# mila-iqia/babyai

Hardware: AMD Instinct MI355X
Metric: env-steps/sec (higher is better)
Workload: dtype u8; 1 GPU; BabyAI-BossLevel-v0 56x56x3 pixel (RGBImgPartialObsWrapper) obs, 1048576 envs in total = 1048576 per GPU x 1, random actions, auto-reset; envs_per_gpu=1048576, total_envs=1048576, parallelism=env-shards x1, no collective

## Files before the change

babyai_amd/csrc/bbai_engine.hip:

```cpp
#include <hip/hip_runtime.h>
#include <stdio.h>
#include <string.h>
#include <stdlib.h>
#include <algorithm>
#include <vector>

#if defined(BBAI_BOT_PROF)
__device__ unsigned long long g_bot_prof[32];
#endif
#include "../../include/bbai.h"
#include "bbai_types.hpp"
#include "bbai_kernels.hpp"
#include "bbai_gen.hpp"
#include "bbai_genl.hpp"
#include "bbai_step.hpp"
#include "bbai_view.hpp"
#include "bbai_grid.hpp"
#include "bbai_bot.hpp"
#include "bbai_seed.hpp"

using namespace bbai;

static_assert(sizeof(bbai_level_cfg) == sizeof(LevelCfg), "C ABI cfg mirrors bbai::LevelCfg");

// ... 79 lines not shown
    hipEvent_t ev_refill[NWIN];
    int gate_strict;
    volatile uint32_t* host_flags;
    uint32_t* host_flags_dev;
    hipStream_t probed[8];
    bool probed_ok[8];
    int n_probed;
    int gate_probe;
    int gate_forced;
    hipStream_t last_stream;
    bool have_stream;
    hipEvent_t ev_switch;
    bool call_events;
    int render_tpb;
    int render_group;
    int pregen_cap;
    int pregen_per_group;
    int pregen_min;
    int pregen_group;
    unsigned long long* tap_mask; uint32_t* tap_rank0; int32_t* tap_perm; int64_t* tap_ids; int64_t tap_count;
    uint32_t* mtt;
    uint8_t* mtpar;
    uint8_t* lane_tmpl;
    int lane_words;
    int pregen_lane;
    int lane_blocks;
    int step_prio;
    bool prof_on;
    struct ProfSlot { hipEvent_t a, b; bool used; } prof[3][PROF_RING];
    int prof_pos[3];
    double prof_ms[3];
    int64_t prof_n[3];
    int64_t prof_step_ticks;
    int rollout_multi;
    int64_t tick;
    uint8_t* vplane;
    uint16_t* fcache;
    uint8_t* cplane;
    uint8_t* lsm;
    unsigned int* render_tickets;
    int render_queue;
    int render_queue_bpc;
    int render_queue_blocks;
    int render_pace;
    uint8_t* rt_pixels;
    uint8_t* rt_shadow;
    bool rt_valid;
    int64_t rt_filled;
    int render_delta;
    int render_delta_sched;
    int render_delta_tpb;
    int render_delta_bpc;
    uint64_t* rt_dmask;
    int render_delta_from_step;
    int n_cus;
    int done_action_enum;
    int consume_fused;
    int inplace;
    uint8_t* atlas;
    uint8_t* lut;
    int n_tiles;
    uint8_t* grid_atlas[3];
    uint8_t* grid_lut[3];
    int grid_tiles[3];
    int grid_bpc;
    bool seeded, live;
    uint8_t* bot_state;
    int bot_stack;
    uint16_t* bot_work;
    uint32_t* bot_rows;
    int bot_group;
    int bot_eager;
    int64_t bot_threads;
    uint64_t* bot_stats;
};

typedef uint32_t u32x4 __attribute__((ext_vector_type(4)));
__device__ __forceinline__ void count_resets(unsigned long long* __restrict__ totals, unsigned int k, unsigned int blk) {
    atomicAdd(&totals[(blk & (SHARDS - 1)) * SHARD_U64], (unsigned long long)k);
}
constexpr int STEP_BLOCK = 64;
#ifndef BBAI_STEP_WAVES
#define BBAI_STEP_WAVES 1
#endif
#ifndef BBAI_PREFETCH_ID
#define BBAI_PREFETCH_ID 0
#endif

#ifndef BBAI_VIEW_LDS
#define BBAI_VIEW_LDS 0
#endif
__device__ __forceinline__ void window_fetch(const uint32_t* __restrict__ q, int rstride, uint32_t* wd) {
#pragma unroll
    for (int r = 0; r < VIEW; ++r) { wd[3 * r] = q[r * rstride]; wd[3 * r + 1] = q[r * rstride + 1]; wd[3 * r + 2] = q[r * rstride + 2]; }
}
__device__ __forceinline__ void view_cells(const uint32_t* wd, int off, int dir, uint32_t ce, int nfe,
                                           uint8_t* __restrict__ scr , uint32_t* cp, uint32_t* vis, int& fe2) {
    uint32_t* win = (uint32_t*)scr;
#pragma unroll
    for (int r = 0; r < VIEW; ++r) {
        win[2 * r] = __builtin_amdgcn_alignbyte(wd[3 * r + 1], wd[3 * r], off);
        win[2 * r + 1] = __builtin_amdgcn_alignbyte(wd[3 * r + 2], wd[3 * r + 1], off);
    }
    const int k0 = dir == 0 ? 6 : dir == 1 ? 54 : dir == 2 ? 48 : 0;
    const int kvi = dir == 0 ? 8 : dir == 1 ? -1 : dir == 2 ? -8 : 1;
    const int kvj = dir == 0 ? -1 : dir == 1 ? -8 : dir == 2 ? 1 : 8;
// ... 1174 lines not shown
    if (threadIdx.x == 0) {
        const unsigned int t0 = atomicAdd(counter, 1u);
        s_ticket[0] = t0;
        s_origin = __builtin_amdgcn_s_memrealtime() * 160ull - ((unsigned long long)t0 * NC + cidx) * (unsigned long long)pace_x16;
    }
    __syncthreads();
    for (;;) {
        const int64_t sg = (int64_t)s_ticket[tp] * NC + cidx;
        if (sg >= n_super) break;
        if (pace_x16) {
            const unsigned long long due = s_origin + (unsigned long long)sg * (unsigned long long)pace_x16;
            while (__builtin_amdgcn_s_memrealtime() * 160ull < due) __builtin_amdgcn_s_sleep(1);
        }
#pragma unroll
        for (int kk = 0; kk < K; ++kk) {
            const int64_t grp = sg * K + kk;
            if (grp >= all_groups) break;
            const int64_t env0 = grp * RENDER_GROUP;
            const int ne = (int)(n - env0 < RENDER_GROUP ? n - env0 : RENDER_GROUP);
            for (int c = threadIdx.x; c < ne * VIEW * VIEW; c += RENDER_BLOCK) {
                const int e = c / (VIEW * VIEW), cell = c - e * (VIEW * VIEW);
                const uint8_t* o = image + (env0 + e) * OBS_BYTES + cell * 3;
                const int key = o[0] | (o[1] << 3) | (o[2] << 6);
                s_tile[buf][c] = s_lut[(cell == 3 * VIEW + 6 ? 256 : 0) + key];
                if (shadow) shadow[env0 * (VIEW * VIEW) + c] = s_tile[buf][c];
            }
            if (kk == 0 && threadIdx.x == 0) s_ticket[tp ^ 1] = atomicAdd(counter, 1u);
            __syncthreads();
            u32x4* out = (u32x4*)(pixels + env0 * PIX_BYTES);
            for (int q = threadIdx.x; q < ne * VEC_PER_ENV; q += RENDER_BLOCK) {
                const int e = q / VEC_PER_ENV, k = q - e * VEC_PER_ENV;
                const uint8_t* t49 = s_tile[buf] + e * (VIEW * VIEW);
                const uint64_t lo = render_chunk(s_atlas, t49, 2 * k);
                const uint64_t hi = render_chunk(s_atlas, t49, 2 * k + 1);
                u32x4 v = {(uint32_t)lo, (uint32_t)(lo >> 32), (uint32_t)hi, (uint32_t)(hi >> 32)};
                __builtin_nontemporal_store(v, out + q);
            }
            buf ^= 1;
        }
        tp ^= 1;
    }
    if (threadIdx.x == 0) {
        unsigned int* departed = counters + 64 * NC;
        if (atomicAdd(departed, 1u) == gridDim.x - 1) {
            for (int c = 0; c <= NC; ++c) atomicExch(counters + 64 * c, 0u);
        }
    }
}

constexpr int LINE_BYTES = 128;
constexpr int DELTA_UNIT = 8;
constexpr int UNIT_LINES = DELTA_UNIT * PIX_BYTES / LINE_BYTES;
static_assert(DELTA_UNIT * PIX_BYTES % LINE_BYTES == 0 && PIX_BYTES % 64 == 0, "8-env units are whole 128-byte lines");

__device__ __forceinline__ uint64_t line_cells(int s, int t) {
    uint64_t m = 0;
    for (int b = s; b < t; b += 8) {
        const int ch = b >> 3, py = ch / CHUNKS_PER_ROW, cx = ch - py * CHUNKS_PER_ROW;
        m |= 1ull << ((cx / 3) * VIEW + (py >> 3));
    }
    return m;
}

template <int G, int T, int SCHED>
__global__ __launch_bounds__(T) void k_render_delta(int64_t n, const uint8_t* __restrict__ image, uint8_t* __restrict__ pixels,
                                                    uint8_t* __restrict__ shadow ,
                                                    const uint8_t* __restrict__ atlas, const uint8_t* __restrict__ lut, int n_tiles) {
    static_assert(G % DELTA_UNIT == 0 && T % 64 == 0 && G % (T / 64) == 0, "whole units per group, whole envs per wave");
    constexpr int W = T / 64, EPW = G / W, GL = G / DELTA_UNIT * UNIT_LINES;
    __shared__ __attribute__((aligned(16))) uint8_t s_atlas[MAX_TILES * TILE_BYTES];
    __shared__ uint64_t s_lma[UNIT_LINES], s_lmb[UNIT_LINES];
    __shared__ uint8_t s_lea[UNIT_LINES];
    __shared__ uint64_t s_dmask[2][G];
    __shared__ uint8_t s_lut[512];
    __shared__ uint8_t s_tile[2][G * CELLS + 8];
    __shared__ uint16_t s_list[2][GL];
    __shared__ unsigned int s_nd[2];
    for (int k = threadIdx.x; k < n_tiles * TILE_BYTES / 8; k += T) ((uint64_t*)s_atlas)[k] = ((const uint64_t*)atlas)[k];
    for (int k = threadIdx.x; k < 512; k += T) s_lut[k] = lut[k];
    for (int l = threadIdx.x; l < UNIT_LINES; l += T) {
        const int b0 = l * LINE_BYTES, b1 = b0 + LINE_BYTES;
        const int ea = b0 / PIX_BYTES, eb = (b1 - 1) / PIX_BYTES;
        s_lea[l] = (uint8_t)ea;
        s_lma[l] = line_cells(b0 - ea * PIX_BYTES, (eb != ea ? (ea + 1) * PIX_BYTES : b1) - ea * PIX_BYTES);
        s_lmb[l] = eb != ea ? line_cells(0, b1 - eb * PIX_BYTES) : 0;
    }
    const int lane = threadIdx.x & 63, wave = threadIdx.x >> 6;
    const int64_t ngroups = (n + G - 1) / G;
    int64_t g, gend, gstep;
    if (SCHED == 0) { g = blockIdx.x; gend = ngroups; gstep = gridDim.x; }
    else { const int64_t per = (ngroups + gridDim.x - 1) / gridDim.x; g = blockIdx.x * per; gend = g + per < ngroups ? g + per : ngroups; gstep = 1; }
    uint32_t o0[EPW], o1[EPW], o2[EPW], old[EPW];
    auto load = [&](int64_t grp) {
#pragma unroll
        for (int j = 0; j < EPW; ++j) {
            const int64_t env = grp * G + wave + j * W;
            o0[j] = o1[j] = o2[j] = old[j] = 0;
            if (grp < gend && lane < CELLS && env < n) {
                const uint8_t* o = image + env * OBS_BYTES + lane * 3;
                o0[j] = o[0]; o1[j] = o[1]; o2[j] = o[2];
                old[j] = shadow[env * CELLS + lane];
            }
        }
    };
    load(g);
    __syncthreads();
    int buf = 0;
    for (; g < gend; g += gstep, buf ^= 1) {
        const int64_t env0 = g * G;
        const int ne = (int)(n - env0 < G ? n - env0 : G);
#pragma unroll
        for (int j = 0; j < EPW; ++j) {
            const int e = wave + j * W;
            const bool live = lane < CELLS && e < ne;
            const int key = o0[j] | (o1[j] << 3) | (o2[j] << 6);
            const uint32_t id = live ? s_lut[(lane == AGENT_CELL ? 256 : 0) + key] : 0;
            const bool d = live && id != old[j];
            const uint64_t m = __ballot(d);
            if (live) s_tile[buf][e * CELLS + lane] = (uint8_t)id;
            if (d) shadow[(env0 + e) * CELLS + lane] = (uint8_t)id;
            if (lane == 0) s_dmask[buf][e] = m;
        }
        if (threadIdx.x == 0) s_nd[buf] = 0;
        __syncthreads();
        const int nl = (int)(((int64_t)ne * PIX_BYTES + LINE_BYTES - 1) / LINE_BYTES);
        for (int L0 = threadIdx.x - lane; L0 < nl; L0 += T) {
            const int L = L0 + lane;
            bool d = false;
            if (L < nl) {
                const int u = L / UNIT_LINES, l = L - u * UNIT_LINES, ea = u * DELTA_UNIT + s_lea[l];
                d = ((s_dmask[buf][ea] & s_lma[l]) | (s_lmb[l] ? s_dmask[buf][ea + 1] & s_lmb[l] : 0)) != 0;
            }
            const uint64_t m = __ballot(d);
            if (!m) continue;
            unsigned int base = 0;
            if (lane == 0) base = atomicAdd(&s_nd[buf], (unsigned int)__builtin_popcountll(m));
            base = __shfl(base, 0);
            if (d) s_list[buf][base + __builtin_popcountll(m & ((1ull << lane) - 1))] = (uint16_t)L;
        }
        __syncthreads();
        const int64_t gn = g + gstep;
        load(gn);
        const int nq = ne * VEC_PER_ENV, nd8 = (int)s_nd[buf] * 8;
        u32x4* out = (u32x4*)(pixels + env0 * PIX_BYTES);
        for (int i = threadIdx.x; i < nd8; i += T) {
            const int q = (int)s_list[buf][i >> 3] * 8 + (i & 7);
            if (q >= nq) continue;
            const int e = q / VEC_PER_ENV, k = q - e * VEC_PER_ENV;
            const uint8_t* t49 = s_tile[buf] + e * CELLS;
            const uint64_t lo = render_chunk(s_atlas, t49, 2 * k);
            const uint64_t hi = render_chunk(s_atlas, t49, 2 * k + 1);
            u32x4 v = {(uint32_t)lo, (uint32_t)(lo >> 32), (uint32_t)hi, (uint32_t)(hi >> 32)};
            __builtin_nontemporal_store(v, out + q);
        }
    }
}

constexpr int DSTORE_PIECES = 32 * CELLS / 8;
template <int G, int T>
__global__ __launch_bounds__(T) void k_render_dstore(int64_t n, uint8_t* __restrict__ pixels, const uint8_t* __restrict__ shadow ,
                                                     const uint64_t* __restrict__ dmask , const uint8_t* __restrict__ atlas, int n_tiles) {
    static_assert(G == 32 && T >= DSTORE_PIECES && T >= G && T % 64 == 0, "one 8-byte shadow piece per thread and group");
    constexpr int GL = G / DELTA_UNIT * UNIT_LINES;
    __shared__ __attribute__((aligned(16))) uint8_t s_atlas[MAX_TILES * TILE_BYTES];
    __shared__ uint64_t s_lma[UNIT_LINES], s_lmb[UNIT_LINES];
    __shared__ uint8_t s_lea[UNIT_LINES];
    __shared__ uint64_t s_dmask[2][G];
    __shared__ __attribute__((aligned(8))) uint8_t s_tile[2][G * CELLS + 8];
    __shared__ uint16_t s_list[2][GL];
    __shared__ unsigned int s_nd[2];
    for (int k = threadIdx.x; k < n_tiles * TILE_BYTES / 8; k += T) ((uint64_t*)s_atlas)[k] = ((const uint64_t*)atlas)[k];
    for (int l = threadIdx.x; l < UNIT_LINES; l += T) {
        const int b0 = l * LINE_BYTES, b1 = b0 + LINE_BYTES;
        const int ea = b0 / PIX_BYTES, eb = (b1 - 1) / PIX_BYTES;
        s_lea[l] = (uint8_t)ea;
        s_lma[l] = line_cells(b0 - ea * PIX_BYTES, (eb != ea ? (ea + 1) * PIX_BYTES : b1) - ea * PIX_BYTES);
        s_lmb[l] = eb != ea ? line_cells(0, b1 - eb * PIX_BYTES) : 0;
    }
    const int tid = threadIdx.x, lane = tid & 63;
    const int64_t ngroups = (n + G - 1) / G;
    const int64_t gstep = gridDim.x;
    int64_t g = blockIdx.x;
    auto load_mask = [&](int64_t grp) -> uint64_t {
        const int64_t env = grp * G + tid;
        return (tid < G && grp < ngroups && env < n) ? dmask[env] : 0ull;
    };
    const uint64_t shared_a = line_cells(PIX_BYTES - LINE_BYTES / 2, PIX_BYTES), shared_b = line_cells(0, LINE_BYTES / 2);
    static_assert(PIX_BYTES % LINE_BYTES == LINE_BYTES / 2, "two envs of a pair share one line");
    auto drawn = [&](int b, int e, int c0, int c1) -> bool {
        if (s_dmask[b][e]) return true;
        const uint64_t pm = (c1 == 63 ? ~0ull : (2ull << c1) - 1) & ~((1ull << c0) - 1);
        const bool shared_stored = ((s_dmask[b][e & ~1] & shared_a) | (s_dmask[b][e | 1] & shared_b)) != 0;
        return shared_stored && (pm & ((e & 1) ? shared_b : shared_a)) != 0;
    };
    auto load_ids = [&](int64_t grp, int b) -> uint2 {
        uint2 r = make_uint2(0u, 0u);
        if (tid >= DSTORE_PIECES || grp >= ngroups) return r;
        const int b0 = 8 * tid, b1 = b0 + 7, ea = b0 / CELLS, eb = b1 / CELLS;
        const bool need = eb == ea ? drawn(b, ea, b0 - ea * CELLS, b1 - ea * CELLS) : (drawn(b, ea, b0 - ea * CELLS, CELLS - 1) || drawn(b, eb, 0, b1 - eb * CELLS));
        if (!need) return r;
        const int64_t base = grp * G * CELLS + 8 * tid, end = n * CELLS;
        if (base + 8 <= end) return *(const uint2*)(shadow + base);
        uint32_t w[2] = {0u, 0u};
        for (int i = 0; i < 8 && base + i < end; ++i) w[i >> 2] |= (uint32_t)shadow[base + i] << (8 * (i & 3));
        return make_uint2(w[0], w[1]);
    };
    if (tid < G) s_dmask[0][tid] = load_mask(g);
    uint64_t mreg = load_mask(g + gstep);
    __syncthreads();
    uint2 idr = load_ids(g, 0);
    int buf = 0;
    for (; g < ngroups; g += gstep, buf ^= 1) {
        const int64_t env0 = g * G;
        const int ne = (int)(n - env0 < G ? n - env0 : G);
        if (tid < DSTORE_PIECES) *(uint2*)(s_tile[buf] + 8 * tid) = idr;
        if (tid < G) s_dmask[buf ^ 1][tid] = mreg;
        if (tid == 0) s_nd[buf] = 0;
        __syncthreads();
        const int nl = (int)(((int64_t)ne * PIX_BYTES + LINE_BYTES - 1) / LINE_BYTES);
        for (int L0 = tid - lane; L0 < nl; L0 += T) {
            const int L = L0 + lane;
            bool d = false;
            if (L < nl) {
                const int u = L / UNIT_LINES, l = L - u * UNIT_LINES, ea = u * DELTA_UNIT + s_lea[l];
                d = ((s_dmask[buf][ea] & s_lma[l]) | (s_lmb[l] ? s_dmask[buf][ea + 1] & s_lmb[l] : 0)) != 0;
            }
            const uint64_t m = __ballot(d);
            if (!m) continue;
            unsigned int base = 0;
            if (lane == 0) base = atomicAdd(&s_nd[buf], (unsigned int)__builtin_popcountll(m));
            base = __shfl(base, 0);
            if (d) s_list[buf][base + __builtin_popcountll(m & ((1ull << lane) - 1))] = (uint16_t)L;
        }
        idr = load_ids(g + gstep, buf ^ 1);
        mreg = load_mask(g + 2 * gstep);
        __syncthreads();
        const int nq = ne * VEC_PER_ENV, nd8 = (int)s_nd[buf] * 8;
        u32x4* out = (u32x4*)(pixels + env0 * PIX_BYTES);
        for (int i = tid; i < nd8; i += T) {
            const int q = (int)s_list[buf][i >> 3] * 8 + (i & 7);
            if (q >= nq) continue;
            const int e = q / VEC_PER_ENV, k = q - e * VEC_PER_ENV;
            const uint8_t* t49 = s_tile[buf] + e * CELLS;
            const uint64_t lo = render_chunk(s_atlas, t49, 2 * k);
            const uint64_t hi = render_chunk(s_atlas, t49, 2 * k + 1);
            u32x4 v = {(uint32_t)lo, (uint32_t)(lo >> 32), (uint32_t)hi, (uint32_t)(hi >> 32)};
            __builtin_nontemporal_store(v, out + q);
        }
    }
}

constexpr int GRID_BLOCK = 1024;
constexpr int GRID_MAX_ENVS = 32;
constexpr int GRID_ID_BYTES = 4096;
constexpr int GRID_MAX_TILES = 132;
constexpr int GRID_UNROLL = 4;

template <int TS> struct GridTile {
    static constexpr int P = TS == 8 ? 8 : 16;
    static constexpr int PPT = TS * 3 / P;
    static constexpr int BYTES = TS * TS * 3;
    static constexpr bool LDS = TS <= 16;
};

struct GridArgs {
    LevelCfg c;
    int64_t n;
    const uint8_t* recs;
    const uint8_t* ring;
    int depth;
    const Hot* hots;
    const int64_t* ids;
    int64_t count;
    uint8_t* out;
    const uint8_t* atlas;
    const uint8_t* lut;
    int n_tiles, highlight;
    int envs_per_item, slices;
    int64_t items;
    uint32_t frame16;
    uint64_t frame_magic;
    uint32_t ppr;
    uint64_t ppr_magic;
};

__device__ __forceinline__ uint32_t grid_div(uint32_t q, uint64_t magic) { return (uint32_t)(((uint64_t)q * magic) >> 32); }

template <int TS>
__device__ __forceinline__ const uint8_t* grid_piece(const uint8_t* atlas, const uint8_t* ids, int W, const GridArgs& a, uint32_t p) {
    using G = GridTile<TS>;
    const uint32_t py = grid_div(p, a.ppr_magic), px = p - py * a.ppr;
    const uint32_t tx = px / G::PPT, part = px - tx * G::PPT;
    const int id = ids[(py / TS) * W + tx];
    return atlas + id * G::BYTES + (py % TS) * (TS * 3) + part * G::P;
}

template <int TS>
__global__ __launch_bounds__(GRID_BLOCK, TS == 16 ? 4 : 8) void k_render_grid(GridArgs a) {
    using G = GridTile<TS>;
    __shared__ __attribute__((aligned(16))) uint8_t s_atlas[G::LDS ? (GRID_MAX_TILES + 1) * G::BYTES : 16];
    __shared__ __attribute__((aligned(16))) uint8_t s_lut[GRID_LUT_BYTES];
// ... 453 lines not shown
        HIP_TRY(hipMemset(e->cplane, 0, (size_t)n_envs * cpl_bytes(c)));
        HIP_TRY(hipMemset(e->fcache, 0, (size_t)n_envs * 2));
    }
    {
        int lo = 0, hi = 0;
        HIP_TRY(hipDeviceGetStreamPriorityRange(&lo, &hi));
        const char* pv = getenv("BBAI_PREGEN_PRIORITY");
        e->side_prio = (pv && atoi(pv) == 0) ? lo : hi;
        HIP_TRY(hipStreamCreateWithPriority(&e->side, hipStreamNonBlocking, e->side_prio));
        e->sides[0] = e->side;
        const char* ls = getenv("BBAI_LOOKAHEAD_STREAMS");
        { int rc = set_sides(e, ls ? atoi(ls) : LOOKAHEAD_STREAMS_DEFAULT); if (rc != BBAI_OK) return rc; }
        HIP_TRY(hipEventCreateWithFlags(&e->ev_consumed, hipEventDisableTiming));
        HIP_TRY(hipStreamCreateWithFlags(&e->split, hipStreamNonBlocking));
        HIP_TRY(hipEventCreateWithFlags(&e->ev_split0, hipEventDisableTiming));
        HIP_TRY(hipEventCreateWithFlags(&e->ev_splitB, hipEventDisableTiming));
        for (int k = 0; k < NWIN; ++k) HIP_TRY(hipEventCreateWithFlags(&e->ev_refill[k], hipEventDisableTiming));
        HIP_TRY(hipEventCreateWithFlags(&e->ev_switch, hipEventDisableTiming));
    }
    {
        const char* cv = getenv("BBAI_CALL_EVENTS");
        e->call_events = cv && atoi(cv) != 0;
        const char* ev = getenv("BBAI_PREGEN_BLOCKS");
        e->pregen_cap = ev ? std::max(64, atoi(ev)) : 16384;
        const char* mv = getenv("BBAI_PREGEN_MIN");
        e->pregen_min = mv ? std::max(0, atoi(mv)) : 6144;
        const char* pp = getenv("BBAI_PREGEN_PER_GROUP");
        e->pregen_per_group = pp ? std::max(1, atoi(pp)) : 12;
        const char* pg = getenv("BBAI_PREGEN_GROUP");
        e->pregen_group = pg ? atoi(pg) : 32;
        const char* sp = getenv("BBAI_STEP_PRIO");
        e->step_prio = sp ? atoi(sp) : 1;
        const char* rv = getenv("BBAI_RENDER_GROUP");
        e->render_group = rv ? atoi(rv) : 0;
        const char* qv = getenv("BBAI_RENDER_QUEUE");
        e->render_queue = qv ? atoi(qv) : -1;
        const char* pv2 = getenv("BBAI_RENDER_PACE");
        e->render_pace = pv2 ? std::max(0, atoi(pv2)) : 0;
        const char* ss = getenv("BBAI_STEP_RENDER_SPLIT");
        e->step_render_split = ss ? atoi(ss) : -1;
        const char* rm = getenv("BBAI_ROLLOUT_MULTI");
        e->rollout_multi = rm ? atoi(rm) : 1;
        const char* gs = getenv("BBAI_GATE_STRICT");
        e->gate_strict = gs ? atoi(gs) != 0 : 0;
        const char* gp = getenv("BBAI_GATE_PROBE");
        e->gate_probe = gp ? atoi(gp) : 1;
        const char* cf = getenv("BBAI_CONSUME_FUSED");
        e->consume_fused = cf ? atoi(cf) : -1;
        const char* tv = getenv("BBAI_RENDER_TPB");
        e->render_tpb = tv ? atoi(tv) : 0;
        const char* dv = getenv("BBAI_RENDER_DELTA");
        e->render_delta = dv ? atoi(dv) != 0 : 1;
        e->render_delta_from_step = -1;
    }
    return BBAI_OK;
}

extern "C" {

void bbai_destroy(bbai_env* e) {
    if (!e) return;
    DeviceGuard guard_(e->device);
    (void)hipDeviceSynchronize();
    if (e->side) (void)hipStreamDestroy(e->side);
    for (int k = 1; k < MAX_SIDES; ++k) if (e->sides[k]) (void)hipStreamDestroy(e->sides[k]);
    if (e->mark_stream) (void)hipStreamDestroy(e->mark_stream);
    for (int k = 0; k < MAX_SIDES; ++k) if (e->ev_part[k]) (void)hipEventDestroy(e->ev_part[k]);
    for (int k = 1; k < MAX_SIDES; ++k) { if (e->gen_lists[k]) (void)hipFree(e->gen_lists[k]); if (e->gen_counts[k]) (void)hipFree(e->gen_counts[k]); }
    if (e->split) (void)hipStreamDestroy(e->split);
    if (e->ev_split0) (void)hipEventDestroy(e->ev_split0);
    if (e->ev_splitB) (void)hipEventDestroy(e->ev_splitB);
    if (e->ev_consumed) (void)hipEventDestroy(e->ev_consumed);
    if (e->ev_switch) (void)hipEventDestroy(e->ev_switch);
    for (int k = 0; k < NWIN; ++k) if (e->ev_refill[k]) (void)hipEventDestroy(e->ev_refill[k]);
    for (int k = 0; k < 3; ++k) for (int i = 0; i < PROF_RING; ++i) if (e->prof[k][i].a) { (void)hipEventDestroy(e->prof[k][i].a); (void)hipEventDestroy(e->prof[k][i].b); }
    void* bot_ptrs[] = {e->bot_state, e->bot_work, e->bot_stats, e->bot_rows};
    for (void* p : bot_ptrs) if (p) (void)hipFree(p);
    void* ptrs[] = {e->rec, e->hot, e->stale, e->mt, e->mti, e->vhead, e->vset, e->next_rec, e->next_hot, e->pending, e->first_slot, e->win_meta, e->totals, e->flow, e->gen_list, e->gen_count, e->reset_list, e->counters,
                    e->atlas, e->lut, e->vplane, e->fcache, e->lsm, e->render_tickets, e->reset_slot, e->next_obs, e->cplane, e->mtt, e->mtpar, e->lane_tmpl, e->tap_mask, e->tap_rank0, e->tap_perm, e->tap_ids, e->rt_shadow, e->rt_dmask};
    for (void* p : ptrs) if (p) (void)hipFree(p);
    for (int k = 0; k < 3; ++k) { if (e->grid_atlas[k]) (void)hipFree(e->grid_atlas[k]); if (e->grid_lut[k]) (void)hipFree(e->grid_lut[k]); }
    if (e->host_flags) (void)hipHostFree((void*)e->host_flags);
    delete e;
}

}

template <int G>
static void launch_pregen_g(const bbai_env* e, unsigned groups, bool listed , uint8_t* pending, const uint8_t* first_slot, int side) {
    unsigned long long* fails = e->flow + FLOW_GEN_FAILURES;
    const dim3 g((groups + 64 / G - 1) / (64 / G)), b(64);
    const int min_groups = e->cfg.num_rows * e->cfg.num_cols > 1 ? 0 : e->pregen_min;
#define PREGEN_LAUNCH(KK, OO) hipLaunchKernelGGL((k_pregen<KK, G, OO>), g, b, 0, e->sides[side], e->cfg, e->n, e->next_rec, e->next_hot, e->mt, e->mti, e->gen_lists[side], \
                                                listed ? e->gen_counts[side] : nullptr, e->depth, pending, first_slot, fails, min_groups, e->pregen_per_group, e->next_obs)
    if (e->cfg.kind == K_LEVELGEN) { if (e->next_obs) PREGEN_LAUNCH(K_LEVELGEN, true); else PREGEN_LAUNCH(K_LEVELGEN, false); }
    else if (e->cfg.kind == K_BONUS) { if (e->next_obs) PREGEN_LAUNCH(K_BONUS, true); else PREGEN_LAUNCH(K_BONUS, false); }
    else { if (e->next_obs) PREGEN_LAUNCH(K_GOTO, true); else PREGEN_LAUNCH(K_GOTO, false); }
#undef PREGEN_LAUNCH
}
static void launch_pregen_lane(const bbai_env* e, int64_t entries_hint, bool listed, uint8_t* pending, const uint8_t* first_slot, int side) {
    LaneLaunch a;
    a.cfg = e->cfg; a.n = e->n; a.next_rec = e->next_rec; a.next_hot = e->next_hot; a.mt = e->mt; a.mtt = e->mtt; a.mtpar = e->mtpar; a.mti = e->mti;
    a.gen_list = e->gen_lists[side]; a.gen_count = listed ? e->gen_counts[side] : nullptr; a.depth = e->depth; a.pending = pending; a.first_slot = first_slot;
    a.fails = e->flow + FLOW_GEN_FAILURES; a.next_obs = e->next_obs; a.tmpl = e->lane_tmpl; a.lane_words = e->lane_words;
    a.blocks = (unsigned)std::max<int64_t>(1, std::min<int64_t>((entries_hint + 63) / 64, e->lane_blocks));
    a.stream = e->sides[side];
// ... 368 lines not shown
    if (pixels && !e->rt_dmask) HIP_TRY(hipMalloc((void**)&e->rt_dmask, (size_t)e->n * sizeof(uint64_t)));
    e->rt_pixels = pixels;
    e->rt_valid = false; e->rt_filled = 0;
    return BBAI_OK;
}

int bbai_render_invalidate(bbai_env* e) {
    if (!e) ARG_FAIL("null handle");
    e->rt_valid = false; e->rt_filled = 0;
    return BBAI_OK;
}

int bbai_render_shadow(bbai_env* e, uint8_t* out, void* stream) {
    if (!e || !out) ARG_FAIL("null handle or buffer");
    if (!e->rt_shadow) { snprintf(g_err, sizeof(g_err), "render_shadow before bbai_set_render_target"); return BBAI_ERR_STATE; }
    ON_DEVICE(e->device);
    hipStream_t s = (hipStream_t)stream;
    CallScope call(e, s);
    if (call.rc != BBAI_OK) return call.rc;
    HIP_TRY(hipMemcpyAsync(out, e->rt_shadow, (size_t)e->n * CELLS, hipMemcpyDeviceToDevice, s));
    return call.leave();
}

}

static bool delta_target(const bbai_env* e, const uint8_t* pixels, int64_t env_off, int64_t nr) {
    const uint8_t* const rt = e->rt_pixels;
    const bool on_target = rt && pixels == rt + env_off * (int64_t)PIX_BYTES && env_off >= 0 && env_off + nr <= e->n;
    return on_target && e->render_delta && e->rt_shadow && ((uintptr_t)rt % LINE_BYTES) == 0 && env_off % DELTA_UNIT == 0;
}
static int render_launch(bbai_env* e, const uint8_t* input, uint8_t* pixels, void* stream, int64_t n_render = -1 ,
                         int64_t env_off = 0 ,
                         bool from_step = false ) {
    CallScope call(e, (hipStream_t)stream);
    if (call.rc != BBAI_OK) return call.rc;
    const int64_t nr = n_render < 0 ? e->n : n_render;
    {
    ProfScope prof_(e, 2, (hipStream_t)stream);
    uint8_t* const rt = e->rt_pixels;
    const int64_t pb = PIX_BYTES;
    const bool delta = delta_target(e, pixels, env_off, nr);
    if (rt && !delta && pixels < rt + e->n * pb && pixels + nr * pb > rt) { e->rt_valid = false; e->rt_filled = 0; }
    uint8_t* const shadow = delta && !e->rt_valid ? e->rt_shadow + env_off * CELLS : nullptr;
    if (shadow && env_off == e->rt_filled) e->rt_filled = env_off + nr;
    if (shadow && e->rt_filled >= e->n) e->rt_valid = true;
    if (delta && !shadow) {
        const int cus = e->n_cus > 0 ? e->n_cus : 256;
        const int T = e->render_delta_tpb == 1024 && !from_step ? 1024 : 512;
        constexpr int G = 32;
        const int64_t groups = (nr + G - 1) / G;
        const int64_t want = (int64_t)cus * (e->render_delta_bpc > 0 ? e->render_delta_bpc : (T == 512 ? 3 : 1));
        const unsigned blocks = (unsigned)std::max<int64_t>(1, std::min<int64_t>(want, groups));
        uint8_t* sh = e->rt_shadow + env_off * CELLS;
        if (from_step) {
            hipLaunchKernelGGL((k_render_dstore<G, 512>), dim3(blocks), dim3(512), 0, (hipStream_t)stream, nr, pixels, sh, e->rt_dmask + env_off, e->atlas, e->n_tiles);
            HIP_TRY(hipGetLastError());
            return call.leave();
        }
#define RENDER_D(TT, SS) hipLaunchKernelGGL((k_render_delta<G, TT, SS>), dim3(blocks), dim3(TT), 0, (hipStream_t)stream, nr, input, pixels, sh, \
                                            e->atlas, e->lut, e->n_tiles)
        if (T == 512) { if (e->render_delta_sched == 1) RENDER_D(512, 1); else RENDER_D(512, 0); }
        else { if (e->render_delta_sched == 1) RENDER_D(1024, 1); else RENDER_D(1024, 0); }
#undef RENDER_D
        HIP_TRY(hipGetLastError());
        return call.leave();
    }
    const bool big = e->n >= 786432;
    int qm = e->render_queue;
    int pace = e->render_pace;
    if (qm < 0) {
        qm = e->n >= RENDER_QUEUE_MIN_ENVS ? RENDER_QUEUE_DEFAULT : 0;
        if (qm == RENDER_QUEUE_DEFAULT && pace > 0) qm = RENDER_QUEUE_PACED;
    }
    if (pace < 0) pace = 0;
    if (qm > 0) {
        const int cus = e->n_cus > 0 ? e->n_cus : 256;
#define RENDER_Q(GG, TT, NC, KK) do { \
            const int64_t tickets = ((nr + GG - 1) / GG + KK - 1) / KK; \
            const int64_t want = e->render_queue_blocks > 0 ? e->render_queue_blocks : (e->render_queue_bpc > 0 ? (int64_t)cus * e->render_queue_bpc : (int64_t)cus * 1024 / TT); \
            const unsigned blocks = (unsigned)std::max<int64_t>(1, std::min<int64_t>(want, tickets)); \
            hipLaunchKernelGGL((k_render_q<GG, TT, NC, KK>), dim3(blocks), dim3(TT), 0, (hipStream_t)stream, nr, input, pixels, \
                               e->atlas, e->lut, e->n_tiles, e->render_tickets, pace, shadow); } while (0)
        switch (qm) {
        default:
        case 1: RENDER_Q(8, 1024, 1, 1); break;
        case 2: RENDER_Q(8, 1024, 8, 1); break;
        case 3: RENDER_Q(8, 1024, 2, 1); break;
        case 4: RENDER_Q(8, 1024, 1, 2); break;
        case 5: RENDER_Q(12, 1024, 1, 1); break;
        case 6: RENDER_Q(16, 1024, 1, 1); break;
        case 7: RENDER_Q(8, 512, 1, 1); break;
        case 8: RENDER_Q(8, 256, 1, 1); break;
        case 9: RENDER_Q(2, 512, 8, 1); break;
        case 10: RENDER_Q(9, 1024, 1, 1); break;
        case 11: RENDER_Q(10, 1024, 1, 1); break;
        }
#undef RENDER_Q
        HIP_TRY(hipGetLastError());
        return call.leave();
    }
    int G = e->render_group, T = e->render_tpb;
    if (G != 2 && G != 4 && G != 8) G = big ? 8 : 2;
    if (T != 256 && T != 512 && T != 1024) T = big ? 1024 : 512;
    const dim3 grid((unsigned)((nr + G - 1) / G));
#define RENDER_LAUNCH(GG, TT) hipLaunchKernelGGL((k_render<GG, TT>), grid, dim3(TT), 0, (hipStream_t)stream, nr, input, pixels, e->atlas, e->lut, e->n_tiles, shadow)
#define RENDER_G(GG) do { if (T == 1024) RENDER_LAUNCH(GG, 1024); else if (T == 512) RENDER_LAUNCH(GG, 512); else RENDER_LAUNCH(GG, 256); } while (0)
    if (G == 2) RENDER_G(2); else if (G == 4) RENDER_G(4); else RENDER_G(8);
#undef RENDER_G
#undef RENDER_LAUNCH
    }
    HIP_TRY(hipGetLastError());
    return call.leave();
}

extern "C" {
// ... 608 lines not shown
        }
    }
    return BBAI_OK;
}

int bbai_gae(int64_t num_envs, int num_frames, const float* rewards, const float* values, const float* masks, const float* last_mask,
             const float* last_value, double discount, double gae_lambda, float* advantage, float* returnn, void* stream) {
    if (num_envs <= 0 || num_frames <= 0 || !rewards || !values || !masks || !last_mask || !last_value || !advantage || !returnn)
        ARG_FAIL("null pointer or empty rollout");
    hipLaunchKernelGGL(k_gae, dim3((unsigned)((num_envs + 63) / 64)), dim3(64), 0, (hipStream_t)stream, num_envs, num_frames, rewards, values,
                       masks, last_mask, last_value, (float)discount, (float)(discount * gae_lambda), advantage, returnn);
    HIP_TRY(hipGetLastError());
    return BBAI_OK;
}

int bbai_set_call_events(bbai_env* e, int enable) {
    if (!e) ARG_FAIL("null handle");
    if (enable && !e->call_events && e->have_stream) {
        ON_DEVICE(e->device);
        HIP_TRY(hipEventRecord(e->ev_switch, e->last_stream));
    }
    e->call_events = enable != 0;
    return BBAI_OK;
}


int bbai_set_done_actions(bbai_env* e, int enable) {
    if (!e) ARG_FAIL("null handle");
    ON_DEVICE(e->device);
    HIP_TRY(hipDeviceSynchronize());
    if (enable && !e->lsm) HIP_TRY(hipMalloc((void**)&e->lsm, (size_t)e->n));
    if (!enable && e->lsm) { HIP_TRY(hipFree(e->lsm)); e->lsm = nullptr; }
    if (e->lsm) HIP_TRY(hipMemset(e->lsm, 0, (size_t)e->n));
    return BBAI_OK;
}
int bbai_get_done_actions(bbai_env* e) { return e && e->lsm ? 1 : 0; }

int bbai_set_option(bbai_env* e, const char* name, int64_t value) {
    if (!e || !name) ARG_FAIL("null handle or name");
    ON_DEVICE(e->device);
    HIP_TRY(hipDeviceSynchronize());
    const int v = (int)value;
    if (!strcmp(name, "render_queue")) e->render_queue = v;
    else if (!strcmp(name, "render_queue_bpc")) e->render_queue_bpc = v;
    else if (!strcmp(name, "render_queue_blocks")) e->render_queue_blocks = v;
    else if (!strcmp(name, "render_pace")) e->render_pace = v < 0 ? 0 : v;
    else if (!strcmp(name, "render_group")) e->render_group = v;
    else if (!strcmp(name, "render_tpb")) e->render_tpb = v;
    else if (!strcmp(name, "render_delta")) { e->render_delta = v != 0; e->rt_valid = false; e->rt_filled = 0; }
    else if (!strcmp(name, "render_delta_sched")) e->render_delta_sched = v;
    else if (!strcmp(name, "render_delta_tpb")) e->render_delta_tpb = v;
    else if (!strcmp(name, "render_delta_bpc")) e->render_delta_bpc = std::max(0, v);
    else if (!strcmp(name, "render_delta_from_step")) e->render_delta_from_step = v < 0 ? -1 : v != 0;
    else if (!strcmp(name, "grid_render_bpc")) e->grid_bpc = std::max(0, v);
    else if (!strcmp(name, "step_prio")) e->step_prio = v;
    else if (!strcmp(name, "pregen_group")) e->pregen_group = v;
    else if (!strcmp(name, "pregen_lane")) {
        if (!e->mtt) { if (v) ARG_FAIL("pregen_lane: this level kind / layout is not covered by the lane generator"); }
        else if ((v != 0) != (e->pregen_lane != 0)) {
            HIP_TRY(hipDeviceSynchronize());
            { int rc = mt_canon(e); if (rc != BBAI_OK) return rc; }
            { int rc = mt_sync(e); if (rc != BBAI_OK) return rc; }
            e->pregen_lane = v != 0;
        }
    }
    else if (!strcmp(name, "lane_blocks")) e->lane_blocks = std::max(1, v);
    else if (!strcmp(name, "pregen_blocks")) e->pregen_cap = std::max(64, v);
    else if (!strcmp(name, "pregen_min")) e->pregen_min = std::max(0, v);
    else if (!strcmp(name, "pregen_per_group")) e->pregen_per_group = std::max(1, v);
    else if (!strcmp(name, "consume_fused")) e->consume_fused = v;
    else if (!strcmp(name, "gate_strict")) e->gate_strict = v != 0;
    else if (!strcmp(name, "gate_probe")) { e->gate_probe = v; e->n_probed = 0; e->gate_forced = 0; }
    else if (!strcmp(name, "gate_fault_inject")) e->host_flags[0] = v != 0;
    else if (!strcmp(name, "bot_group")) e->bot_group = v;
    else if (!strcmp(name, "step_render_split")) e->step_render_split = v;
    else if (!strcmp(name, "rollout_multi")) e->rollout_multi = v;
    else if (!strcmp(name, "lookahead_streams")) { int rc = set_sides(e, v); if (rc != BBAI_OK) return rc; }
    else if (!strcmp(name, "done_action_enum")) e->done_action_enum = v != 0;
    else {
        snprintf(g_err, sizeof(g_err), "set_option: unknown option '%s'", name);
        return BBAI_ERR_ARG;
    }
    return BBAI_OK;
}

static int read_flow(bbai_env* e, int word, unsigned long long* out) {
    HIP_TRY(hipDeviceSynchronize());
    HIP_TRY(hipMemcpy(out, e->flow + word, 8, hipMemcpyDeviceToHost));
    return BBAI_OK;
}

int bbai_get_option(bbai_env* e, const char* name, int64_t* out) {
    if (!e || !name || !out) ARG_FAIL("null handle, name or output");
    if (!strcmp(name, "render_queue")) *out = e->render_queue;
    else if (!strcmp(name, "render_queue_bpc")) *out = e->render_queue_bpc;
    else if (!strcmp(name, "render_queue_blocks")) *out = e->render_queue_blocks;
    else if (!strcmp(name, "render_pace")) *out = e->render_pace;
    else if (!strcmp(name, "render_group")) *out = e->render_group;
    else if (!strcmp(name, "render_tpb")) *out = e->render_tpb;
    else if (!strcmp(name, "render_delta")) *out = e->render_delta;
    else if (!strcmp(name, "render_delta_sched")) *out = e->render_delta_sched;
    else if (!strcmp(name, "render_delta_tpb")) *out = e->render_delta_tpb;
    else if (!strcmp(name, "render_delta_bpc")) *out = e->render_delta_bpc;
    else if (!strcmp(name, "render_delta_from_step")) *out = e->render_delta_from_step;
    else if (!strcmp(name, "grid_render_bpc")) *out = e->grid_bpc;
    else if (!strcmp(name, "render_delta_valid")) *out = e->rt_valid ? 1 : 0;
    else if (!strcmp(name, "step_prio")) *out = e->step_prio;
    else if (!strcmp(name, "pregen_group")) *out = e->pregen_group;
    else if (!strcmp(name, "pregen_lane")) *out = e->pregen_lane;
    else if (!strcmp(name, "lane_blocks")) *out = e->lane_blocks;
    else if (!strcmp(name, "pregen_blocks")) *out = e->pregen_cap;
    else if (!strcmp(name, "pregen_min")) *out = e->pregen_min;
    else if (!strcmp(name, "pregen_per_group")) *out = e->pregen_per_group;
    else if (!strcmp(name, "consume_fused")) *out = e->consume_fused;
    else if (!strcmp(name, "gate_strict")) *out = e->gate_strict;
    else if (!strcmp(name, "gate_probe")) *out = e->gate_probe;
    else if (!strcmp(name, "gate_forced_strict")) *out = e->gate_forced;
    else if (!strcmp(name, "gate_fault")) *out = e->host_flags ? (int64_t)e->host_flags[0] : 0;
    else if (!strcmp(name, "bot_group")) *out = e->bot_group;
    else if (!strcmp(name, "step_render_split")) *out = e->step_render_split;
    else if (!strcmp(name, "rollout_multi")) *out = e->rollout_multi;
    else if (!strcmp(name, "lookahead_streams")) *out = e->n_sides;
    else if (!strcmp(name, "profile_step_ticks")) *out = e->prof_step_ticks;
    else if (!strcmp(name, "inplace")) *out = e->inplace;
    else if (!strcmp(name, "cplane")) *out = e->cplane ? 1 : 0;
    else if (!strcmp(name, "done_action_enum")) *out = e->done_action_enum;
    else if (!strcmp(name, "lookahead_period")) *out = e->period;
    else if (!strcmp(name, "gate_timeouts")) {
        ON_DEVICE(e->device);
        unsigned long long v = 0;
        int rc = read_flow(e, FLOW_GATE_TIMEOUTS, &v);
        if (rc != BBAI_OK) return rc;
        *out = (int64_t)v;
    }
    else if (!strcmp(name, "render_pace_effective")) *out = e->render_pace > 0 ? e->render_pace : 0;
    else {
        snprintf(g_err, sizeof(g_err), "get_option: unknown option '%s'", name);
        return BBAI_ERR_ARG;
    }
    return BBAI_OK;
}

int bbai_profile(bbai_env* e, int enable) {
    if (!e) ARG_FAIL("null handle");
    e->prof_on = enable != 0;
    if (enable == 1) e->prof_step_ticks = 0;
    if (enable == 1) for (int k = 0; k < 3; ++k) { e->prof_ms[k] = 0; e->prof_n[k] = 0; for (int i = 0; i < PROF_RING; ++i) e->prof[k][i].used = false; }
    return BBAI_OK;
}

int bbai_profile_read(bbai_env* e, double* ms_total , int64_t* launches ) {
    if (!e || !ms_total || !launches) ARG_FAIL("null pointer");
    ON_DEVICE(e->device);
    for (int k = 0; k < 3; ++k) {
        for (int i = 0; i < PROF_RING; ++i) prof_fold(e, k, i);
        ms_total[k] = e->prof_ms[k]; launches[k] = e->prof_n[k];
    }
// ... 25 lines not shown
```

Before: 1.542 billion env-steps/s.

## Render dirty 64-byte pixel pieces per wave instead of 128-byte group lines

Adds a piece-granular delta render path, with 64 bytes as the new default. Each wave builds its own list of dirty pieces per env from a cell mask and re-renders only those pieces. Block-wide syncs and the shared group line list are replaced with wave-local LDS syncs, and the dstore variant pipelines the mask and shadow loads across a triple buffer. This cuts redundant pixel writes for unchanged cells and block synchronisation, at the cost of smaller store granularity and per-env wave-serial work. The 128-byte line path stays available through an option.

```diff
diff --git a/babyai_amd/csrc/bbai_engine.hip b/babyai_amd/csrc/bbai_engine.hip
--- a/babyai_amd/csrc/bbai_engine.hip
+++ b/babyai_amd/csrc/bbai_engine.hip
@@ -155,6 +155,7 @@
     int render_delta_tpb;
     int render_delta_bpc;
     uint64_t* rt_dmask;
+    int render_piece_bytes;
     int render_delta_from_step;
     int n_cus;
     int done_action_enum;
@@ -1435,6 +1436,7 @@
 constexpr int DELTA_UNIT = 8;
 constexpr int UNIT_LINES = DELTA_UNIT * PIX_BYTES / LINE_BYTES;
 static_assert(DELTA_UNIT * PIX_BYTES % LINE_BYTES == 0 && PIX_BYTES % 64 == 0, "8-env units are whole 128-byte lines");
+constexpr int RENDER_PIECE_DEFAULT = 64;
 
 __device__ __forceinline__ uint64_t line_cells(int s, int t) {
     uint64_t m = 0;
@@ -1445,29 +1447,56 @@
     return m;
 }
 
-template <int G, int T, int SCHED>
+template <int P>
+struct Pieces {
+    static_assert(P == 16 || P == 32 || P == 64, "pieces of 16, 32 or 64 bytes");
+    static_assert(PIX_BYTES % P == 0, "whole pieces per env");
+    static constexpr int NP = PIX_BYTES / P;
+    static constexpr int S = P / 16;
+};
+
+__device__ __forceinline__ void wave_lds_sync() {
+    __builtin_amdgcn_fence(__ATOMIC_RELEASE, "workgroup");
+    __builtin_amdgcn_wave_barrier();
+    __builtin_amdgcn_fence(__ATOMIC_ACQUIRE, "workgroup");
+}
+
+template <int P>
+__device__ __forceinline__ void init_piece_cells(uint64_t* s_pm, int tid, int nthreads) {
+    for (int p = tid; p < Pieces<P>::NP; p += nthreads) s_pm[p] = line_cells(p * P, p * P + P);
+}
+
+template <int P>
+__device__ __forceinline__ void store_dirty_pieces(uint64_t m, const uint64_t* s_pm, uint16_t* wl, const uint8_t* s_atlas, const uint8_t* t49,
+                                                   u32x4* out, int lane) {
+    constexpr int NP = Pieces<P>::NP, S = Pieces<P>::S;
+    int cnt = 0;
+    for (int p0 = 0; p0 < NP; p0 += 64) {
+        const int p = p0 + lane;
+        const bool d = p < NP && (m & s_pm[p]) != 0;
+        const uint64_t b = __ballot(d);
+        if (d) wl[cnt + __builtin_popcountll(b & ((1ull << lane) - 1))] = (uint16_t)p;
+        cnt += __builtin_popcountll(b);
+    }
+    wave_lds_sync();
+    for (int i = lane; i < cnt * S; i += 64) {
+        const int k = (int)wl[i / S] * S + (i & (S - 1));
+        const uint64_t lo = render_chunk(s_atlas, t49, 2 * k);
+        const uint64_t hi = render_chunk(s_atlas, t49, 2 * k + 1);
+        u32x4 v = {(uint32_t)lo, (uint32_t)(lo >> 32), (uint32_t)hi, (uint32_t)(hi >> 32)};
+        __builtin_nontemporal_store(v, out + k);
+    }
+    wave_lds_sync();
+}
+
+template <int G, int T, int SCHED, int P>
 __global__ __launch_bounds__(T) void k_render_delta(int64_t n, const uint8_t* __restrict__ image, uint8_t* __restrict__ pixels,
                                                     uint8_t* __restrict__ shadow ,
                                                     const uint8_t* __restrict__ atlas, const uint8_t* __restrict__ lut, int n_tiles) {
     static_assert(G % DELTA_UNIT == 0 && T % 64 == 0 && G % (T / 64) == 0, "whole units per group, whole envs per wave");
     constexpr int W = T / 64, EPW = G / W, GL = G / DELTA_UNIT * UNIT_LINES;
     __shared__ __attribute__((aligned(16))) uint8_t s_atlas[MAX_TILES * TILE_BYTES];
-    __shared__ uint64_t s_lma[UNIT_LINES], s_lmb[UNIT_LINES];
-    __shared__ uint8_t s_lea[UNIT_LINES];
-    __shared__ uint64_t s_dmask[2][G];
     __shared__ uint8_t s_lut[512];
-    __shared__ uint8_t s_tile[2][G * CELLS + 8];
-    __shared__ uint16_t s_list[2][GL];
-    __shared__ unsigned int s_nd[2];
-    for (int k = threadIdx.x; k < n_tiles * TILE_BYTES / 8; k += T) ((uint64_t*)s_atlas)[k] = ((const uint64_t*)atlas)[k];
-    for (int k = threadIdx.x; k < 512; k += T) s_lut[k] = lut[k];
-    for (int l = threadIdx.x; l < UNIT_LINES; l += T) {
-        const int b0 = l * LINE_BYTES, b1 = b0 + LINE_BYTES;
-        const int ea = b0 / PIX_BYTES, eb = (b1 - 1) / PIX_BYTES;
-        s_lea[l] = (uint8_t)ea;
-        s_lma[l] = line_cells(b0 - ea * PIX_BYTES, (eb != ea ? (ea + 1) * PIX_BYTES : b1) - ea * PIX_BYTES);
-        s_lmb[l] = eb != ea ? line_cells(0, b1 - eb * PIX_BYTES) : 0;
-    }
     const int lane = threadIdx.x & 63, wave = threadIdx.x >> 6;
     const int64_t ngroups = (n + G - 1) / G;
     int64_t g, gend, gstep;
@@ -1486,6 +1515,53 @@
             }
         }
     };
+    for (int k = threadIdx.x; k < n_tiles * TILE_BYTES / 8; k += T) ((uint64_t*)s_atlas)[k] = ((const uint64_t*)atlas)[k];
+    for (int k = threadIdx.x; k < 512; k += T) s_lut[k] = lut[k];
+    if constexpr (P < LINE_BYTES) {
+        __shared__ uint64_t s_pm[Pieces<P>::NP];
+        __shared__ uint16_t s_wl[W][Pieces<P>::NP];
+        __shared__ uint8_t s_tile1[G * CELLS + 8];
+        init_piece_cells<P>(s_pm, threadIdx.x, T);
+        load(g);
+        __syncthreads();
+        for (; g < gend; g += gstep) {
+            const int64_t env0 = g * G;
+            const int ne = (int)(n - env0 < G ? n - env0 : G);
+            uint64_t dm[EPW];
+#pragma unroll
+            for (int j = 0; j < EPW; ++j) {
+                const int e = wave + j * W;
+                const bool live = lane < CELLS && e < ne;
+                const int key = o0[j] | (o1[j] << 3) | (o2[j] << 6);
+                const uint32_t id = live ? s_lut[(lane == AGENT_CELL ? 256 : 0) + key] : 0;
+                const bool d = live && id != old[j];
+                dm[j] = __ballot(d);
+                if (live) s_tile1[e * CELLS + lane] = (uint8_t)id;
+                if (d) shadow[(env0 + e) * CELLS + lane] = (uint8_t)id;
+            }
+            load(g + gstep);
+            wave_lds_sync();
+#pragma unroll
+            for (int j = 0; j < EPW; ++j) {
+                const int e = wave + j * W;
+                if (dm[j]) store_dirty_pieces<P>(dm[j], s_pm, s_wl[wave], s_atlas, s_tile1 + e * CELLS, (u32x4*)(pixels + (env0 + e) * PIX_BYTES), lane);
+            }
+        }
+        return;
+    } else {
+    __shared__ uint64_t s_lma[UNIT_LINES], s_lmb[UNIT_LINES];
+    __shared__ uint8_t s_lea[UNIT_LINES];
+    __shared__ uint64_t s_dmask[2][G];
+    __shared__ uint8_t s_tile[2][G * CELLS + 8];
+    __shared__ uint16_t s_list[2][GL];
+    __shared__ unsigned int s_nd[2];
+    for (int l = threadIdx.x; l < UNIT_LINES; l += T) {
+        const int b0 = l * LINE_BYTES, b1 = b0 + LINE_BYTES;
+        const int ea = b0 / PIX_BYTES, eb = (b1 - 1) / PIX_BYTES;
+        s_lea[l] = (uint8_t)ea;
+        s_lma[l] = line_cells(b0 - ea * PIX_BYTES, (eb != ea ? (ea + 1) * PIX_BYTES : b1) - ea * PIX_BYTES);
+        s_lmb[l] = eb != ea ? line_cells(0, b1 - eb * PIX_BYTES) : 0;
+    }
     load(g);
     __syncthreads();
     int buf = 0;
@@ -1537,29 +1613,18 @@
             __builtin_nontemporal_store(v, out + q);
         }
     }
+    }
 }
 
 constexpr int DSTORE_PIECES = 32 * CELLS / 8;
-template <int G, int T>
+template <int G, int T, int P>
 __global__ __launch_bounds__(T) void k_render_dstore(int64_t n, uint8_t* __restrict__ pixels, const uint8_t* __restrict__ shadow ,
                                                      const uint64_t* __restrict__ dmask , const uint8_t* __restrict__ atlas, int n_tiles) {
     static_assert(G == 32 && T >= DSTORE_PIECES && T >= G && T % 64 == 0, "one 8-byte shadow piece per thread and group");
     constexpr int GL = G / DELTA_UNIT * UNIT_LINES;
     __shared__ __attribute__((aligned(16))) uint8_t s_atlas[MAX_TILES * TILE_BYTES];
-    __shared__ uint64_t s_lma[UNIT_LINES], s_lmb[UNIT_LINES];
-    __shared__ uint8_t s_lea[UNIT_LINES];
-    __shared__ uint64_t s_dmask[2][G];
     __shared__ __attribute__((aligned(8))) uint8_t s_tile[2][G * CELLS + 8];
-    __shared__ uint16_t s_list[2][GL];
-    __shared__ unsigned int s_nd[2];
     for (int k = threadIdx.x; k < n_tiles * TILE_BYTES / 8; k += T) ((uint64_t*)s_atlas)[k] = ((const uint64_t*)atlas)[k];
-    for (int l = threadIdx.x; l < UNIT_LINES; l += T) {
-        const int b0 = l * LINE_BYTES, b1 = b0 + LINE_BYTES;
-        const int ea = b0 / PIX_BYTES, eb = (b1 - 1) / PIX_BYTES;
-        s_lea[l] = (uint8_t)ea;
-        s_lma[l] = line_cells(b0 - ea * PIX_BYTES, (eb != ea ? (ea + 1) * PIX_BYTES : b1) - ea * PIX_BYTES);
-        s_lmb[l] = eb != ea ? line_cells(0, b1 - eb * PIX_BYTES) : 0;
-    }
     const int tid = threadIdx.x, lane = tid & 63;
     const int64_t ngroups = (n + G - 1) / G;
     const int64_t gstep = gridDim.x;
@@ -1568,6 +1633,60 @@
         const int64_t env = grp * G + tid;
         return (tid < G && grp < ngroups && env < n) ? dmask[env] : 0ull;
     };
+    auto load_piece = [&](int64_t grp) -> uint2 {
+        const int64_t base = grp * G * CELLS + 8 * tid, end = n * CELLS;
+        if (base + 8 <= end) return *(const uint2*)(shadow + base);
+        uint32_t w[2] = {0u, 0u};
+        for (int i = 0; i < 8 && base + i < end; ++i) w[i >> 2] |= (uint32_t)shadow[base + i] << (8 * (i & 3));
+        return make_uint2(w[0], w[1]);
+    };
+    if constexpr (P < LINE_BYTES) {
+        constexpr int W = T / 64, EPW = G / W;
+        __shared__ uint64_t s_pm[Pieces<P>::NP];
+        __shared__ uint16_t s_wl[W][Pieces<P>::NP];
+        __shared__ uint64_t s_dm3[3][G];
+        const int wave = tid >> 6;
+        init_piece_cells<P>(s_pm, tid, T);
+        auto load_ids = [&](int64_t grp, int b) -> uint2 {
+            if (tid >= DSTORE_PIECES || grp >= ngroups) return make_uint2(0u, 0u);
+            const int ea = (8 * tid) / CELLS, eb = (8 * tid + 7) / CELLS;
+            if (!s_dm3[b][ea] && !s_dm3[b][eb]) return make_uint2(0u, 0u);
+            return load_piece(grp);
+        };
+        if (tid < G) s_dm3[0][tid] = load_mask(g);
+        uint64_t mreg = load_mask(g + gstep);
+        __syncthreads();
+        uint2 idr = load_ids(g, 0);
+        int buf = 0, mb = 0;
+        for (; g < ngroups; g += gstep, buf ^= 1, mb = mb == 2 ? 0 : mb + 1) {
+            const int64_t env0 = g * G;
+            const int mn = mb == 2 ? 0 : mb + 1;
+            if (tid < DSTORE_PIECES) *(uint2*)(s_tile[buf] + 8 * tid) = idr;
+            if (tid < G) s_dm3[mn][tid] = mreg;
+            __syncthreads();
+            idr = load_ids(g + gstep, mn);
+            mreg = load_mask(g + 2 * gstep);
+#pragma unroll
+            for (int j = 0; j < EPW; ++j) {
+                const int e = wave + j * W;
+                const uint64_t m = s_dm3[mb][e];
+                if (m) store_dirty_pieces<P>(m, s_pm, s_wl[wave], s_atlas, s_tile[buf] + e * CELLS, (u32x4*)(pixels + (env0 + e) * PIX_BYTES), lane);
+            }
+        }
+        return;
+    } else {
+    __shared__ uint64_t s_lma[UNIT_LINES], s_lmb[UNIT_LINES];
+    __shared__ uint8_t s_lea[UNIT_LINES];
+    __shared__ uint64_t s_dmask[2][G];
+    __shared__ uint16_t s_list[2][GL];
+    __shared__ unsigned int s_nd[2];
+    for (int l = threadIdx.x; l < UNIT_LINES; l += T) {
+        const int b0 = l * LINE_BYTES, b1 = b0 + LINE_BYTES;
+        const int ea = b0 / PIX_BYTES, eb = (b1 - 1) / PIX_BYTES;
+        s_lea[l] = (uint8_t)ea;
+        s_lma[l] = line_cells(b0 - ea * PIX_BYTES, (eb != ea ? (ea + 1) * PIX_BYTES : b1) - ea * PIX_BYTES);
+        s_lmb[l] = eb != ea ? line_cells(0, b1 - eb * PIX_BYTES) : 0;
+    }
     const uint64_t shared_a = line_cells(PIX_BYTES - LINE_BYTES / 2, PIX_BYTES), shared_b = line_cells(0, LINE_BYTES / 2);
     static_assert(PIX_BYTES % LINE_BYTES == LINE_BYTES / 2, "two envs of a pair share one line");
     auto drawn = [&](int b, int e, int c0, int c1) -> bool {
@@ -1582,11 +1701,7 @@
         const int b0 = 8 * tid, b1 = b0 + 7, ea = b0 / CELLS, eb = b1 / CELLS;
         const bool need = eb == ea ? drawn(b, ea, b0 - ea * CELLS, b1 - ea * CELLS) : (drawn(b, ea, b0 - ea * CELLS, CELLS - 1) || drawn(b, eb, 0, b1 - eb * CELLS));
         if (!need) return r;
-        const int64_t base = grp * G * CELLS + 8 * tid, end = n * CELLS;
-        if (base + 8 <= end) return *(const uint2*)(shadow + base);
-        uint32_t w[2] = {0u, 0u};
-        for (int i = 0; i < 8 && base + i < end; ++i) w[i >> 2] |= (uint32_t)shadow[base + i] << (8 * (i & 3));
-        return make_uint2(w[0], w[1]);
+        return load_piece(grp);
     };
     if (tid < G) s_dmask[0][tid] = load_mask(g);
     uint64_t mreg = load_mask(g + gstep);
@@ -1630,6 +1745,7 @@
             u32x4 v = {(uint32_t)lo, (uint32_t)(lo >> 32), (uint32_t)hi, (uint32_t)(hi >> 32)};
             __builtin_nontemporal_store(v, out + q);
         }
+    }
     }
 }
 
@@ -2189,6 +2305,7 @@
         const char* dv = getenv("BBAI_RENDER_DELTA");
         e->render_delta = dv ? atoi(dv) != 0 : 1;
         e->render_delta_from_step = -1;
+        e->render_piece_bytes = RENDER_PIECE_DEFAULT;
     }
     return BBAI_OK;
 }
@@ -2663,15 +2780,21 @@
         const int64_t want = (int64_t)cus * (e->render_delta_bpc > 0 ? e->render_delta_bpc : (T == 512 ? 3 : 1));
         const unsigned blocks = (unsigned)std::max<int64_t>(1, std::min<int64_t>(want, groups));
         uint8_t* sh = e->rt_shadow + env_off * CELLS;
+        const int pb = e->render_piece_bytes;
         if (from_step) {
-            hipLaunchKernelGGL((k_render_dstore<G, 512>), dim3(blocks), dim3(512), 0, (hipStream_t)stream, nr, pixels, sh, e->rt_dmask + env_off, e->atlas, e->n_tiles);
+#define RENDER_S(PP) hipLaunchKernelGGL((k_render_dstore<G, 512, PP>), dim3(blocks), dim3(512), 0, (hipStream_t)stream, nr, pixels, sh, e->rt_dmask + env_off, \
+                                        e->atlas, e->n_tiles)
+            if (pb == 128) RENDER_S(128); else RENDER_S(64);
+#undef RENDER_S
             HIP_TRY(hipGetLastError());
             return call.leave();
         }
-#define RENDER_D(TT, SS) hipLaunchKernelGGL((k_render_delta<G, TT, SS>), dim3(blocks), dim3(TT), 0, (hipStream_t)stream, nr, input, pixels, sh, \
-                                            e->atlas, e->lut, e->n_tiles)
-        if (T == 512) { if (e->render_delta_sched == 1) RENDER_D(512, 1); else RENDER_D(512, 0); }
-        else { if (e->render_delta_sched == 1) RENDER_D(1024, 1); else RENDER_D(1024, 0); }
+#define RENDER_D(TT, SS, PP) hipLaunchKernelGGL((k_render_delta<G, TT, SS, PP>), dim3(blocks), dim3(TT), 0, (hipStream_t)stream, nr, input, pixels, sh, \
+                                                e->atlas, e->lut, e->n_tiles)
+#define RENDER_DP(TT, SS) do { if (pb == 128) RENDER_D(TT, SS, 128); else RENDER_D(TT, SS, 64); } while (0)
+        if (T == 512) { if (e->render_delta_sched == 1) RENDER_DP(512, 1); else RENDER_DP(512, 0); }
+        else { if (e->render_delta_sched == 1) RENDER_DP(1024, 1); else RENDER_DP(1024, 0); }
+#undef RENDER_DP
 #undef RENDER_D
         HIP_TRY(hipGetLastError());
         return call.leave();
@@ -3386,6 +3509,10 @@
     else if (!strcmp(name, "render_delta_tpb")) e->render_delta_tpb = v;
     else if (!strcmp(name, "render_delta_bpc")) e->render_delta_bpc = std::max(0, v);
     else if (!strcmp(name, "render_delta_from_step")) e->render_delta_from_step = v < 0 ? -1 : v != 0;
+    else if (!strcmp(name, "render_piece_bytes")) {
+        if (v != 64 && v != 128) ARG_FAIL("render_piece_bytes: 64 or 128");
+        e->render_piece_bytes = v;
+    }
     else if (!strcmp(name, "grid_render_bpc")) e->grid_bpc = std::max(0, v);
     else if (!strcmp(name, "step_prio")) e->step_prio = v;
     else if (!strcmp(name, "pregen_group")) e->pregen_group = v;
@@ -3437,6 +3564,7 @@
     else if (!strcmp(name, "render_delta_tpb")) *out = e->render_delta_tpb;
     else if (!strcmp(name, "render_delta_bpc")) *out = e->render_delta_bpc;
     else if (!strcmp(name, "render_delta_from_step")) *out = e->render_delta_from_step;
+    else if (!strcmp(name, "render_piece_bytes")) *out = e->render_piece_bytes;
     else if (!strcmp(name, "grid_render_bpc")) *out = e->grid_bpc;
     else if (!strcmp(name, "render_delta_valid")) *out = e->rt_valid ? 1 : 0;
     else if (!strcmp(name, "step_prio")) *out = e->step_prio;
```

Result: faster. 1.587 billion env-steps/s (median of 6 runs) (+2.9%).
